# heliaxdev/ark-plonk

Measured on AMD Instinct MI355X. Metric: proofs/sec at 2^20 constraints (BLS12-381, KZG10); MSM G1-adds/s, higher is better.
Workload: dtype u32 limbs (256/384-bit Montgomery integers)

## Files before the change

### ark_plonk_amd/context.py

```python
from __future__ import annotations

import ctypes
import os
import threading

import numpy as np

from . import _lib
from ._lib import check, lib

_default = {}
_default_lock = threading.Lock()


def _is_torch(x) -> bool:
    return type(x).__module__.startswith("torch")


class Context:

    def __init__(self, device: int = 0, stream=None):
        self._h = ctypes.c_void_p()
        check(lib().zk_ctx_create(int(device), ctypes.byref(self._h)), "zk_ctx_create")
        self.device = int(device)
        self._stream_ptr = None
        self._stream_thread = None
        if stream is not None:
            self.set_stream(stream)
        lws = int(os.environ.get("LOCAL_WORLD_SIZE", "1") or 1)
        if lws > 1:
            cores = len(os.sched_getaffinity(0)) if hasattr(os, "sched_getaffinity") else (os.cpu_count() or 1)
            self.set_option("host_workers", max(0, min(15, cores // lws - 1)))

    def close(self):
        if getattr(self, "_h", None) is not None and self._h:
            lib().zk_ctx_destroy(self._h)
            self._h = None

    def __del__(self):
        try:
            self.close()
        except Exception:
            pass

    @property
    def handle(self):
        if not self._h:
            raise RuntimeError("context closed")
        return self._h

    def set_stream(self, stream):
        if stream is None:
            check(lib().zk_ctx_use_own_stream(self.handle), "zk_ctx_use_own_stream")
            self._stream_ptr = None
            self._stream_thread = None
            return
        ptr = int(getattr(stream, "cuda_stream", stream))
        if self._stream_ptr == ptr:
            return
        me = threading.get_ident()
        if self._stream_thread not in (None, me) and self._stream_ptr is not None:
            raise RuntimeError("Context is bound to another thread's stream: use one Context per thread and stream "
                               "(contexts are cheap and share CommitterKey handles via CommitterKey.with_ctx)")
        check(lib().zk_ctx_set_stream(self.handle, ctypes.c_void_p(ptr)), "zk_ctx_set_stream")
        self._stream_ptr = ptr
        self._stream_thread = me

    def use_torch_stream(self):
        import torch
        self.set_stream(torch.cuda.current_stream(self.device))

    def sync(self):
        check(lib().zk_ctx_sync(self.handle), "zk_ctx_sync")

    def set_msm_window(self, c: int):
        check(lib().zk_ctx_set_msm_window(self.handle, int(c)), "zk_ctx_set_msm_window")

    OPTIONS = ("msm_merge", "pre_vw", "pre_logg", "chunk_l", "long_rounds", "combine_sg", "pre_max_log_n", "mem_reserve_mb",
               "round_mem_limit_mb", "host_workers", "cache_verify")

    def set_option(self, key: str, value: int):
        check(lib().zk_ctx_set_option(self.handle, key.encode(), int(value)), f"zk_ctx_set_option({key})")

    def get_option(self, key: str) -> int:
        v = ctypes.c_int64()
        check(lib().zk_ctx_get_option(self.handle, key.encode(), ctypes.byref(v)), f"zk_ctx_get_option({key})")
        return v.value

    def round_mem_stats(self) -> dict:
        v = [ctypes.c_uint64() for _ in range(4)]
        check(lib().zk_round_mem_stats(self.handle, *[ctypes.byref(x) for x in v]), "zk_round_mem_stats")
        return {"early_closes": v[0].value, "set_bytes": v[1].value, "device_free": v[2].value, "device_total": v[3].value}

    def set_commit_cache(self, on: bool = True, capacity: int = 0):
        check(lib().zk_ctx_set_commit_cache(self.handle, 1 if on else 0, int(capacity)), "zk_ctx_set_commit_cache")

    def commit_cache_stats(self) -> dict:
        v = [ctypes.c_uint64() for _ in range(3)]
        check(lib().zk_commit_cache_stats(self.handle, *[ctypes.byref(x) for x in v]), "zk_commit_cache_stats")
        return {"hits": v[0].value, "misses": v[1].value, "entries": v[2].value}

    def set_residency_cache(self, on: bool = True, capacity_bytes: int = 0, max_vector_bytes: int = 0):
        check(lib().zk_ctx_set_residency_cache(self.handle, 1 if on else 0, int(capacity_bytes), int(max_vector_bytes)), "zk_ctx_set_residency_cache")

    def residency_cache_stats(self) -> dict:
        v = [ctypes.c_uint64() for _ in range(4)]
        check(lib().zk_residency_cache_stats(self.handle, *[ctypes.byref(x) for x in v]), "zk_residency_cache_stats")
        return {"hits": v[0].value, "misses": v[1].value, "entries": v[2].value, "bytes": v[3].value}

    def cache_verify_stats(self) -> dict:
        a, b = ctypes.c_uint64(), ctypes.c_uint64()
        check(lib().zk_cache_verify_stats(self.handle, ctypes.byref(a), ctypes.byref(b)), "zk_cache_verify_stats")
        return {"checked": a.value, "mismatches": b.value}

    def io_stats(self, reset: bool = False) -> dict:
        a, b = ctypes.c_uint64(), ctypes.c_uint64()
        check(lib().zk_io_stats(self.handle, ctypes.byref(a), ctypes.byref(b), 1 if reset else 0), "zk_io_stats")
        return {"h2d_bytes": a.value, "d2h_bytes": b.value}

    def set_staging(self, pinned_ring: bool = False):
        check(lib().zk_ctx_set_staging(self.handle, 1 if pinned_ring else 0), "zk_ctx_set_staging")

    def profile(self, on=True):
        check(lib().zk_profile_enable(self.handle, int(on)))

    def profile_reset(self):
        check(lib().zk_profile_reset(self.handle))

    def profile_get(self, name: str):
        t = ctypes.c_double()
        n = ctypes.c_uint64()
        check(lib().zk_profile_get(self.handle, name.encode(), ctypes.byref(t), ctypes.byref(n)))
        return t.value, n.value


def default_context(device: int = 0) -> Context:
    with _default_lock:
        ctx = _default.get(device)
        if ctx is None:
            ctx = Context(device)
            _default[device] = ctx
        return ctx


def ptr_of(x):
    if _is_torch(x):
        return ctypes.c_void_p(x.data_ptr())
    return ctypes.c_void_p(x.ctypes.data)


def as_host_u64(x, cols: int) -> np.ndarray:
    a = np.ascontiguousarray(x, dtype=np.uint64)
    if a.size % cols:
        raise ValueError(f"array size {a.size} not a multiple of {cols} limbs")
    return a.reshape(-1, cols)


def check_dev_tensor(t, cols: int, device: int):
    import torch
    if not t.is_cuda:
        raise ValueError("expected a CUDA/HIP tensor")
    if t.device.index != device:
# ... 9 lines not shown
```

### ark_plonk_amd/csrc/api_ctx.hip

```cpp
#include "api_internal.h"

#include <cstdio>

static thread_local char g_last_hip[256];

void zk_note_hip_error(hipError_t e, const char* what, const char* file, int line) {
    snprintf(g_last_hip, sizeof g_last_hip, "%s (%s) at %s:%d", hipGetErrorString(e), what, file, line);
    if (getenv("ZK_VERBOSE")) fprintf(stderr, "[ark_plonk_amd] HIP error: %s\n", g_last_hip);
}

ProfScope::ProfScope(zk_ctx* ctx, const char* nm) : ProfScope(ctx, nm, ctx->stream) {}
ProfScope::ProfScope(zk_ctx* ctx, const char* nm, hipStream_t stream) : c(ctx), name(nm), st(stream) {
    if (!c->profiling) return;
    if (c->profile_level == 2 && strcmp(nm, "msm_accumulate") != 0) return;
    auto take = [&]() -> hipEvent_t {
        if (!c->event_pool.empty()) {
            hipEvent_t e = c->event_pool.back();
            c->event_pool.pop_back();
            return e;
        }
        hipEvent_t e = nullptr;
        (void)hipEventCreate(&e);
        return e;
    };
// ... 65 lines not shown
    if (e != hipSuccess) {
        delete c;
        (void)hipSetDevice(prev);
        return ZK_ERR_HIP;
    }
    c->stream = c->own_stream;
    {
        const unsigned hc = std::thread::hardware_concurrency();
        c->tune.host_workers = hc > 16 ? 15 : hc > 1 ? (int)hc - 1 : 0;
        c->pool.reset(new HostPool((unsigned)c->tune.host_workers));
    }
    c->key_from_os = zk_process_key(c->ccache.digest_key);
    c->ccache.digest_key[0] ^= (uint64_t)(uintptr_t)c * 0x9E3779B97F4A7C15ull;
    for (int i = 0; i < ZK_MAX_JOBS && e == hipSuccess; ++i) e = hipEventCreateWithFlags(&c->ev_job[i], hipEventDisableTiming);
    (void)hipSetDevice(prev);
    if (e != hipSuccess) {
        zk_ctx_destroy(c);
        return ZK_ERR_HIP;
    }
    *out = c;
    return ZK_OK;
}

void zk_ctx_destroy(zk_ctx* c) {
    if (!c) return;
    {
        Guard g(c);
        (void)hipStreamSynchronize(c->stream);
        zk_prof_collect(c);
        for (hipEvent_t e : c->event_pool) (void)hipEventDestroy(e);
        ntt_ctx_free(c);
        DevBuf* bufs[] = {&c->io.a, &c->io.b, &c->msm_tmp, &c->stage_shared, &c->witness};
        for (DevBuf* b : bufs) b->release();
        for (int i = 0; i < ZK_MAX_JOBS; ++i) c->mb[i].release();
        res_clear(c);
        for (int i = 0; i < ZK_MAX_JOBS; ++i)
            if (c->ev_job[i]) (void)hipEventDestroy(c->ev_job[i]);
        if (c->round.ev) (void)hipEventDestroy(c->round.ev);
        if (c->pinned) (void)hipHostFree(c->pinned);
        if (c->pinned_small) (void)hipHostFree(c->pinned_small);
        if (c->round.pinned_jobs) (void)hipHostFree(c->round.pinned_jobs);
        zk_io_release(c);
        if (c->own_stream) (void)hipStreamDestroy(c->own_stream);
    }
    delete c;
}

static int switch_stream(zk_ctx* c, hipStream_t st) {
    Guard g(c);
    ZK_HIP_TRY(hipStreamSynchronize(c->stream));
    c->stream = st;
    return ZK_OK;
}
int zk_ctx_set_stream(zk_ctx* c, void* hip_stream) { return c ? switch_stream(c, (hipStream_t)hip_stream) : ZK_ERR_BAD_ARG; }
int zk_ctx_use_own_stream(zk_ctx* c) { return c ? switch_stream(c, c->own_stream) : ZK_ERR_BAD_ARG; }

int zk_ctx_sync(zk_ctx* c) {
    if (!c) return ZK_ERR_BAD_ARG;
    Guard g(c);
    ZK_HIP_TRY(hipStreamSynchronize(c->stream));
    return ZK_OK;
}

int zk_ctx_set_msm_window(zk_ctx* c, int w) {
    if (!c || w < 0 || w > 16 || w == 1) return ZK_ERR_BAD_ARG;
    Guard g(c);
    if (round_open(c)) return ZK_ERR_PENDING;
    c->msm_window = w;
    return ZK_OK;
}

static int* tune_field(zk_ctx* c, const char* key, int64_t* lo, int64_t* hi) {
    struct Row {
        const char* key;
        int ZkTune::*field;
        int64_t lo, hi;
    };
    static const Row rows[] = {
        {"msm_merge", &ZkTune::msm_merge, 0, 1},         {"pre_vw", &ZkTune::pre_vw, 0, 512},
        {"pre_logg", &ZkTune::pre_logg, -1, 5},          {"chunk_l", &ZkTune::chunk_l, 0, 1024},
        {"long_rounds", &ZkTune::long_rounds, 1, 16},    {"combine_sg", &ZkTune::combine_sg, 0, 4},
        {"pre_max_log_n", &ZkTune::pre_max_log_n, 0, 25}, {"mem_reserve_mb", &ZkTune::mem_reserve_mb, 0, 1 << 20},
        {"round_mem_limit_mb", &ZkTune::round_mem_limit_mb, 0, 1 << 20},
    };
    for (const Row& r : rows)
        if (strcmp(key, r.key) == 0) {
            *lo = r.lo;
            *hi = r.hi;
            return &(c->tune.*(r.field));
        }
    return nullptr;
}

int zk_ctx_set_option(zk_ctx* c, const char* key, int64_t value) {
    if (!c || !key) return ZK_ERR_BAD_ARG;
    Guard g(c);
    if (round_open(c)) return ZK_ERR_PENDING;
    int64_t lo = 0, hi = 0;
    if (strcmp(key, "cache_verify") == 0) {
        if (value < 0 || value > 1) return ZK_ERR_BAD_ARG;
        c->cache_verify = value != 0;
        return ZK_OK;
    }
    if (strcmp(key, "host_workers") == 0) {
        if (value < 0 || value > 63) return ZK_ERR_BAD_ARG;
        c->pool.reset(new HostPool((unsigned)value));
        c->tune.host_workers = (int)value;
        return ZK_OK;
    }
    int* f = tune_field(c, key, &lo, &hi);
    if (!f) return ZK_ERR_UNSUPPORTED;
    if (value < lo || value > hi) return ZK_ERR_BAD_ARG;
    if (f == &c->tune.pre_vw && value && (value < 8 || (value & (value - 1)))) return ZK_ERR_BAD_ARG;
    if (f == &c->tune.chunk_l && value && value < 8) return ZK_ERR_BAD_ARG;
    if (f == &c->tune.combine_sg && value == 3) return ZK_ERR_BAD_ARG;
    if (f == &c->tune.pre_max_log_n && value && value < 13) return ZK_ERR_BAD_ARG;
    *f = (int)value;
    return ZK_OK;
}

int zk_ctx_get_option(zk_ctx* c, const char* key, int64_t* value) {
    if (!c || !key || !value) return ZK_ERR_BAD_ARG;
    Guard g(c);
    int64_t lo = 0, hi = 0;
    if (strcmp(key, "host_workers") == 0) {
        *value = c->tune.host_workers;
        return ZK_OK;
    }
    if (strcmp(key, "cache_verify") == 0) {
        *value = c->cache_verify ? 1 : 0;
        return ZK_OK;
    }
    int* f = tune_field(c, key, &lo, &hi);
    if (!f) return ZK_ERR_UNSUPPORTED;
    *value = *f;
    return ZK_OK;
}

int zk_cache_verify_stats(zk_ctx* c, uint64_t* checked, uint64_t* mismatches) {
    if (!c) return ZK_ERR_BAD_ARG;
    Guard g(c);
    if (checked) *checked = c->verify_checked;
    if (mismatches) *mismatches = c->verify_mismatch;
    return ZK_OK;
}

int zk_profile_enable(zk_ctx* c, int on) {
    if (!c) return ZK_ERR_BAD_ARG;
    Guard g(c);
    c->profiling = on != 0;
    c->profile_level = on;
    return ZK_OK;
}
int zk_profile_reset(zk_ctx* c) {
    if (!c) return ZK_ERR_BAD_ARG;
    Guard g(c);
    ZK_HIP_TRY(hipStreamSynchronize(c->stream));
    zk_prof_collect(c);
    for (auto& kv : c->prof) {
        kv.second.total_ms = 0;
        kv.second.launches = 0;
    }
    return ZK_OK;
}
int zk_profile_get(zk_ctx* c, const char* name, double* total_ms, uint64_t* launches) {
    if (!c || !name) return ZK_ERR_BAD_ARG;
// ... 57 lines not shown
```

### ark_plonk_amd/csrc/ctx.h

```cpp
#pragma once
#include <hip/hip_runtime.h>
#include <cstring>
#include <cstdlib>
#include <atomic>
#include <list>
#include <map>
#include <mutex>
#include <shared_mutex>
#include <string>
#include <thread>
#include <condition_variable>
#include <functional>
#include <memory>
#include <vector>
#include <utility>

#include "../../include/ark_plonk_amd.h"
#include "curve_params.h"
#include "ec.cuh"
#include "fieldu.cuh"
#include "ecu.cuh"

typedef Fp<FrBls12_381Params> FrBls;
typedef Fp<FqBls12_381Params> FqBls;
// ... 131 lines not shown
    size_t need_for(size_t bytes) const { return bytes <= cap ? 0 : want_for(bytes); }
    int ensure(size_t bytes) {
        if (bytes <= cap) return ZK_OK;
        if (p) (void)hipFree(p);
        p = nullptr;
        cap = 0;
        size_t want = want_for(bytes);
        hipError_t e = hipMalloc(&p, want);
        if (e != hipSuccess) {
            p = nullptr;
            return ZK_ERR_OOM;
        }
        cap = want;
        return ZK_OK;
    }
    void release() {
        if (p) (void)hipFree(p);
        p = nullptr;
        cap = 0;
    }
};

struct MsmBufs {
    DevBuf counts, offsets, entries, buckets, part_pt, part_key, seg, seg2, seg3, win, tmp, scalars, stage, upload;
    int stage_of_job = 0;
    uint32_t acc_chunk_l = 0, acc_n_lanes = 0;
    void release() {
        release_work();
        scalars.release();
        upload.release();
    }
    void work_bufs(DevBuf* (&out)[12]) {
        DevBuf* all[12] = {&counts, &offsets, &entries, &buckets, &part_pt, &part_key, &seg, &seg2, &seg3, &win, &tmp, &stage};
        for (int i = 0; i < 12; ++i) out[i] = all[i];
    }
    size_t work_bytes() {
        DevBuf* w[12];
        work_bufs(w);
        size_t t = 0;
        for (DevBuf* b : w) t += b->cap;
        return t;
    }
    void release_work() {
        DevBuf* w[12];
        work_bufs(w);
        for (DevBuf* b : w) b->release();
    }
    void swap_work(MsmBufs& o) {
        DevBuf* a[12];
        DevBuf* b[12];
        work_bufs(a);
        o.work_bufs(b);
        for (int i = 0; i < 12; ++i) std::swap(*a[i], *b[i]);
    }
};

struct ProfEntry {
    double total_ms = 0;
    uint64_t launches = 0;
    std::vector<std::pair<hipEvent_t, hipEvent_t>> pending;
};

struct NttPlan {
    int curve = 0;
    uint32_t log_n = 0;
    bool inverse = false;
    int n_pass = 0;
    int s[4] = {0, 0, 0, 0};
    void* tw_inner[4] = {nullptr, nullptr, nullptr, nullptr};
    void* tw_pass[4] = {nullptr, nullptr, nullptr, nullptr};
    ~NttPlan() {
        for (int i = 0; i < 4; ++i)
            if (tw_pass[i]) (void)hipFree(tw_pass[i]);
    }
};

struct ZkTune {
    int msm_merge = 1;
    int pre_vw = 0;
    int pre_logg = -1;
    int chunk_l = 0;
    int long_rounds = 1;
    int combine_sg = 0;
    int pre_max_log_n = 0;
    int mem_reserve_mb = 1024;
    int round_mem_limit_mb = 0;
    int host_workers = -1;
};

struct zk_ctx {
    int device = 0;
    ZkTune tune;
    hipStream_t stream = nullptr;
    hipStream_t own_stream = nullptr;
    std::recursive_mutex mu;
    std::unique_ptr<HostPool> pool;
    int msm_window = 0;
    bool profiling = false;
    int profile_level = 0;
    std::map<std::string, ProfEntry> prof;
    std::vector<hipEvent_t> event_pool;

    std::map<uint64_t, NttPlan*> plans;
    std::map<uint64_t, void*> inner_tw;
    DevBuf ntt_work;
    DevBuf coset_pow[2];
    DevBuf coset_inv_pow[2];
    size_t coset_len[2] = {0, 0};
    size_t coset_inv_len[2] = {0, 0};

    MsmBufs mb[ZK_MAX_JOBS];
    hipEvent_t ev_job[ZK_MAX_JOBS] = {};
    void* pinned = nullptr;
    size_t pinned_cap = 0;
    void* pinned_small = nullptr;
    DevBuf msm_tmp;
    DevBuf stage_shared;
    DevBuf witness;

    struct HostIo {
        DevBuf a, b;
        hipStream_t copy_stream = nullptr;
        static constexpr int STAGE_SLOTS = 4;
        static constexpr size_t STAGE_BYTES = (size_t)8 << 20;
        void* stage_pin[STAGE_SLOTS] = {nullptr, nullptr, nullptr, nullptr};
        hipEvent_t stage_ev[STAGE_SLOTS] = {nullptr, nullptr, nullptr, nullptr};
        bool stage_busy[STAGE_SLOTS] = {false, false, false, false};
        int stage_next = 0;
        hipEvent_t ev_up[ZK_MAX_JOBS] = {};
        uint64_t h2d_bytes = 0, d2h_bytes = 0;
        int staging_mode = 0;
    } io;

    struct CommitCache {
        struct Entry {
            uint64_t srs_id;
            uint64_t n;
            uint32_t kind;
            uint64_t dig[4];
            uint64_t xy[ZK_MAX_AFFINE64];
            uint8_t inf;
        };
        bool on = false;
        size_t cap = 64;
        std::list<Entry> entries;
        uint64_t hits = 0, misses = 0;
        DevBuf digest_dev;
        uint64_t digest_key[4] = {0, 0, 0, 0};
    } ccache;

    struct Residency {
        struct Entry {
            size_t bytes = 0;
            uint64_t dig[4] = {0, 0, 0, 0};
            bool valid = false;
            uint64_t epoch = 0;
            uint64_t born = 0;
            DevBuf buf;
        };
        bool on = false;
        size_t cap = (size_t)2 << 30, max_vec = (size_t)64 << 20, bytes = 0;
        std::list<Entry> entries;
        std::vector<DevBuf> free_bufs;
        uint64_t epoch = 0, hits = 0, misses = 0;
        std::vector<unsigned char> verify_host;
    } res;
// ... 141 lines not shown
```

### ark_plonk_amd/csrc/ecq.cuh

```cuda
#pragma once
#include "ecu.cuh"

template <class F>
ZK_D F quad_xor(const F& v, int mask) {
    F r;
#pragma unroll
    for (int i = 0; i < F::NL; ++i) r.v[i] = __shfl_xor(v.v[i], mask, 64);
    return r;
}
template <class F>
ZK_D F quad_bcast(const F& v, uint32_t src_role) {
    const int src = (int)((__lane_id() & ~3u) | src_role);
    F r;
#pragma unroll
    for (int i = 0; i < F::NL; ++i) r.v[i] = __shfl(v.v[i], src, 64);
    return r;
}
template <class F>
ZK_D F fsel(bool c, const F& a, const F& b) {
    F r;
#pragma unroll
    for (int i = 0; i < F::NL; ++i) r.v[i] = c ? a.v[i] : b.v[i];
    return r;
}
ZK_D bool quad_flag(bool f, uint32_t src_role) {
    const unsigned long long b = __ballot(f);
    return (b >> ((__lane_id() & ~3u) | src_role)) & 1ull;
}

template <class F>
ZK_D XYZZu<F> quad_gather(const F& c) {
    XYZZu<F> p;
    p.x = quad_bcast(c, 0);
    p.y = quad_bcast(c, 1);
    p.zz = quad_bcast(c, 2);
    p.zzz = quad_bcast(c, 3);
    return p;
}
template <class F>
ZK_D F quad_pick(const XYZZu<F>& p, uint32_t role) {
    return role == 0 ? p.x : role == 1 ? p.y : role == 2 ? p.zz : p.zzz;
}
template <class F>
ZK_D bool quad_is_inf(const F& c, uint32_t role) {
    return quad_flag(role == 2 && c.limbs_zero(), 2);
}

template <class F>
ZK_D F qdbl(const F& p, uint32_t role);

template <class F>
ZK_D F qadd(const F& p, const F& q, uint32_t role) {
    const bool p_inf = quad_is_inf(p, role), q_inf = quad_is_inf(q, role);
    const F m1 = F::mul(p, quad_xor(q, 2));
    const F d = F::sub8(quad_xor(m1, 2), m1);
    const bool lo = role < 2;
    const F m2 = F::mul(fsel(lo, d, p), fsel(lo, d, q));
    const F bc_u1 = quad_bcast(m1, 0), bc_pp = quad_bcast(m2, 0);
    const F m3 = F::mul(role == 0 ? d : role == 1 ? bc_u1 : m2, fsel(role == 0, m2, bc_pp));
    const F bc_ppp = quad_bcast(m3, 0);
    const F x3 = F::sub_sum3(m2, bc_ppp, m3, m3);
    const bool r1 = role == 1;
    const F m4 = F::dot2(fsel(r1, d, m2), fsel(r1, F::sub16(m3, x3), bc_ppp), fsel(r1, F::neg16(m1), F::zero()), bc_ppp);
    const F x3_from_role1 = quad_xor(x3, 1);
    F res = role == 0 ? x3_from_role1 : role == 2 ? m3 : m4;
    const bool same_x = quad_flag(role == 2 && m3.is_zero_mod_reduced(), 2);
    const bool same_y = quad_flag(role == 1 && m2.is_zero_mod_reduced(), 1);
    const bool slow = same_x && !p_inf && !q_inf;
    if (__any(slow)) {
        const F twice = qdbl<F>(p, role);
        if (slow) res = same_y ? twice : F::zero();
    }
    if (q_inf) res = p;
    if (p_inf) res = q;
    return res;
}

template <class F>
ZK_D F qdbl(const F& p, uint32_t role) {
    const bool p_inf = quad_is_inf(p, role);
    const F a1 = fsel(role == 1, F::dbl(p), p);
    const F m1 = F::mul(a1, a1);
    const F bc_v = quad_bcast(m1, 1);
    const F m2 = F::mul(a1, bc_v);
    const F mm = F::add3(m1, m1, m1);
    const F bc_w = quad_bcast(m2, 1);
    const bool r0 = role == 0;
    const F m3 = F::mul(fsel(r0, mm, p), fsel(r0, mm, bc_w));
    const F x3 = F::sub8(m3, F::dbl(m2));
    const F m4 = F::dot2(mm, F::sub16(m2, x3), bc_w, F::neg16(quad_bcast(p, 1)));
    const F y3_from_role0 = quad_xor(m4, 1);
    F res = role == 0 ? x3 : role == 1 ? y3_from_role0 : role == 2 ? m2 : m3;
    if (p_inf) res = p;
    return res;
}
```

### ark_plonk_amd/csrc/msm_reduce.hip

```cpp
#include "msm_common.cuh"
#include "ecq.cuh"

namespace {


ZK_D uint64_t partial_slot(uint32_t t, uint32_t ta, uint32_t s, uint32_t L) {
    return (t == ta && (s % L) != 0) ? 2ull * t + 1 : 2ull * t;
}

template <class F>
ZK_D XYZZu<F> wave_sum(XYZZu<F> acc) {
#pragma unroll 1
    for (int d = 32; d >= 1; d >>= 1) {
        XYZZu<F> o;
#pragma unroll
        for (int i = 0; i < F::NL; ++i) {
            o.x.v[i] = __shfl_down(acc.x.v[i], d, 64);
            o.y.v[i] = __shfl_down(acc.y.v[i], d, 64);
            o.zz.v[i] = __shfl_down(acc.zz.v[i], d, 64);
            o.zzz.v[i] = __shfl_down(acc.zzz.v[i], d, 64);
        }
        acc = XYZZu<F>::add(acc, o);
    }
    return acc;
// ... 242 lines not shown
    auto bucket = [&](int i) -> F {
        const uint32_t bi = w * g.B + sg * G + (uint32_t)i;
        F v = F::zero();
        if (live && (!offsets || offsets[bi + 1] != offsets[bi])) v = ld_coord<F>(buckets, bi, role);
        return v;
    };
    F nv = bucket((int)G - 1);
#pragma unroll 1
    for (int i = (int)G - 1; i >= 0; --i) {
        const F v = nv;
        if (i > 0) nv = bucket(i - 1);
        run = qadd<F>(run, v, role);
        acc = qadd<F>(acc, run, role);
    }
    if (live) {
        st_coord<F>(seg_run, id, role, run);
        st_coord<F>(seg_acc, id, role, acc);
    }
}

template <class F, int MAXT>
__global__ void __launch_bounds__(MAXT) __attribute__((amdgpu_waves_per_eu(MAXT / 256, MAXT / 256))) msm_win_finish_q(RJobs jobs, MsmGeom g, uint32_t raw) {
    extern __shared__ uint4 sh[];
    const void* seg_run = jobs.seg_run[blockIdx.y];
    const void* seg_acc = jobs.seg_acc[blockIdx.y];
    uint32_t* win_out = jobs.win_s[blockIdx.y];
    uint32_t* tot_out = jobs.win_t[blockIdx.y];
    const uint32_t w = blockIdx.x, u = threadIdx.x >> 2, role = threadIdx.x & 3;
    const uint32_t T = blockDim.x >> 2;
    F R = F::zero(), Y = F::zero();
    if (u < g.ns) {
        R = ld_coord<F>(seg_run, (uint64_t)w * g.ns + u, role);
        Y = ld_coord<F>(seg_acc, (uint64_t)w * g.ns + u, role);
    }
    st_coord<F>(sh, u, role, R);
    for (uint32_t d = 1; d < T; d <<= 1) {
        __syncthreads();
        F o = F::zero();
        if (u + d < T) o = ld_coord<F>(sh, u + d, role);
        __syncthreads();
        R = qadd<F>(R, o, role);
        st_coord<F>(sh, u, role, R);
    }
    const bool r_inf = quad_is_inf(R, role);
    if (tot_out && u == 0) {
        if (raw) {
            st_coord<F>(tot_out, w, role, r_inf ? F::zero() : R);
        } else {
            uint32_t* o = tot_out + (size_t)w * 4 * F::SAT + role * F::SAT;
            if (r_inf) {
                for (int i = 0; i < F::SAT; ++i) o[i] = 0;
            } else {
                R.to_sat(o);
            }
        }
    }
    F Qm = R;
    for (uint32_t k = 0; k < g.logG; ++k) Qm = qdbl<F>(Qm, role);
    F Z = qadd<F>(Y, u >= 1 ? Qm : F::zero(), role);
    __syncthreads();
    st_coord<F>(sh, u, role, Z);
    for (uint32_t d = T / 2; d >= 1; d >>= 1) {
        __syncthreads();
        if (u < d) {
            Z = qadd<F>(Z, ld_coord<F>(sh, u + d, role), role);
            st_coord<F>(sh, u, role, Z);
        }
    }
    const bool z_inf = quad_is_inf(Z, role);
    if (u == 0) {
        if (raw) {
            st_coord<F>(win_out, w, role, z_inf ? F::zero() : Z);
        } else {
            uint32_t* o = win_out + (size_t)w * 4 * F::SAT + role * F::SAT;
            if (z_inf) {
                for (int i = 0; i < F::SAT; ++i) o[i] = 0;
            } else {
                Z.to_sat(o);
            }
        }
    }
}

template <class F>
__global__ void __launch_bounds__(256) __attribute__((amdgpu_waves_per_eu(1, 2))) msm_node_reduce_q(RJobs jobs, uint32_t n_out, uint32_t logk, uint32_t logm) {
    const void* in_run = jobs.seg_run[blockIdx.y];
    const void* in_acc = jobs.seg_acc[blockIdx.y];
    void* out_run = jobs.win_s[blockIdx.y];
    void* out_acc = jobs.win_t[blockIdx.y];
    const uint32_t tid = blockIdx.x * blockDim.x + threadIdx.x;
    const uint32_t id = tid >> 2, role = tid & 3;
    const bool live = id < n_out;
    const uint32_t K = 1u << logk;
    const uint64_t first = (uint64_t)(live ? id : 0) * K;
    F run = F::zero(), wsum = F::zero(), asum = F::zero();
#pragma unroll 1
    for (int j = (int)K - 1; j >= 1; --j) {
        run = qadd<F>(run, live ? ld_coord<F>(in_run, first + (uint32_t)j, role) : F::zero(), role);
        wsum = qadd<F>(wsum, run, role);
        asum = qadd<F>(asum, live ? ld_coord<F>(in_acc, first + (uint32_t)j, role) : F::zero(), role);
    }
    run = qadd<F>(run, live ? ld_coord<F>(in_run, first, role) : F::zero(), role);
    asum = qadd<F>(asum, live ? ld_coord<F>(in_acc, first, role) : F::zero(), role);
    for (uint32_t t = 0; t < logm; ++t) wsum = qdbl<F>(wsum, role);
    asum = qadd<F>(asum, wsum, role);
    if (live) {
        st_coord<F>(out_run, id, role, run);
        st_coord<F>(out_acc, id, role, asum);
    }
}

template <class F>
__global__ void __launch_bounds__(256) __attribute__((amdgpu_waves_per_eu(1, 2))) g1_sum_winsums_q(const void* all, uint32_t ranks, uint32_t n_pts ,
                                                                                                     uint32_t logq, uint32_t* out_sat) {
    extern __shared__ uint4 sh[];
    const uint32_t Q = 1u << logq;
    const uint32_t quad = threadIdx.x >> 2, role = threadIdx.x & 3;
    const uint32_t per_block = (blockDim.x >> 2) >> logq;
    const uint32_t k = blockIdx.x * per_block + (quad >> logq), j = quad & (Q - 1);
    const bool live = k < n_pts;
    F acc = F::zero();
#pragma unroll 1
    for (uint32_t r = j; r < ranks; r += Q) acc = qadd<F>(acc, live ? ld_coord<F>(all, (uint64_t)r * n_pts + k, role) : F::zero(), role);
    for (uint32_t d = Q >> 1; d >= 1; d >>= 1) {
        st_coord<F>(sh, quad, role, acc);
        __syncthreads();
        const F o = j < d ? ld_coord<F>(sh, quad + d, role) : F::zero();
        __syncthreads();
        acc = qadd<F>(acc, o, role);
    }
    const bool inf = quad_is_inf(acc, role);
    if (live && j == 0) {
        uint32_t* o = out_sat + (size_t)k * 4 * F::SAT + role * F::SAT;
        if (inf) {
            for (int i = 0; i < F::SAT; ++i) o[i] = 0;
        } else {
            acc.to_sat(o);
        }
    }
}

template <class F>
int launch_win_finish_q(dim3 grid, uint32_t chains, hipStream_t st, const RJobs& jobs, const MsmGeom& g, uint32_t raw) {
    constexpr size_t PT = (size_t)4 * Store<F>::WORDS * 4;
    const size_t shmem = (size_t)chains * PT;
    if (chains <= 128) {
        if (shmem > 48 * 1024)
            ZK_HIP_TRY(hipFuncSetAttribute((const void*)msm_win_finish_q<F, 512>, hipFuncAttributeMaxDynamicSharedMemorySize, (int)shmem));
        hipLaunchKernelGGL((msm_win_finish_q<F, 512>), grid, dim3(4 * chains), shmem, st, jobs, g, raw);
    } else if (chains <= 256) {
        if (shmem > 48 * 1024)
            ZK_HIP_TRY(hipFuncSetAttribute((const void*)msm_win_finish_q<F, 1024>, hipFuncAttributeMaxDynamicSharedMemorySize, (int)shmem));
        hipLaunchKernelGGL((msm_win_finish_q<F, 1024>), grid, dim3(4 * chains), shmem, st, jobs, g, raw);
    } else {
        return ZK_ERR_UNSUPPORTED;
    }
    return ZK_OK;
}

template <class F>
int queue_reduce(zk_ctx* c, const RJobs& jobs, uint32_t n_jobs, uint32_t nb, const MsmGeom& gr, hipStream_t st, bool queues_cleared = false,
                 uint32_t raw = 0 ) {
    constexpr size_t PT = (size_t)4 * Store<F>::WORDS * 4;
    ProfScope ps(c, "msm_reduce", st);
    const int T = 128;
    int rc;
    if (!queues_cleared)
        for (uint32_t k = 0; k < n_jobs; ++k) ZK_HIP_TRY(hipMemsetAsync(jobs.q[k], 0, 8, st));
    const bool quad = gr.logq == 0 && gr.ns <= 256;
    if (n_jobs <= 2) {
        if (quad) {
            unsigned blocks = (unsigned)(((uint64_t)nb * 4 + 255) / 256);
            hipLaunchKernelGGL(msm_combine_q<F>, dim3(blocks, n_jobs), dim3(256), 0, st, jobs, nb);
        } else {
            unsigned blocks = (unsigned)(((uint64_t)nb * 4 + T - 1) / T);
            hipLaunchKernelGGL((msm_combine<F, 4>), dim3(blocks, n_jobs), dim3(T), 0, st, jobs, nb);
        }
    } else {
        const int sg = c->tune.combine_sg ? c->tune.combine_sg : 1;
        if (sg == 4) {
            unsigned blocks = (unsigned)(((uint64_t)nb * 4 + T - 1) / T);
            hipLaunchKernelGGL((msm_combine<F, 4>), dim3(blocks, n_jobs), dim3(T), 0, st, jobs, nb);
        } else if (sg == 2) {
            unsigned blocks = (unsigned)(((uint64_t)nb * 2 + T - 1) / T);
            hipLaunchKernelGGL((msm_combine<F, 2>), dim3(blocks, n_jobs), dim3(T), 0, st, jobs, nb);
        } else {
            unsigned blocks = (unsigned)(((uint64_t)nb + T - 1) / T);
            hipLaunchKernelGGL((msm_combine<F, 1>), dim3(blocks, n_jobs), dim3(T), 0, st, jobs, nb);
        }
    }
    hipLaunchKernelGGL(msm_combine_wave<F>, dim3(256, n_jobs), dim3(256), 0, st, jobs);
    hipLaunchKernelGGL(msm_combine_block<F>, dim3(64, n_jobs), dim3(256), 4 * PT, st, jobs, nb);
    if (quad) {
        unsigned sblocks = (unsigned)(((uint64_t)gr.W * gr.ns * 4 + 255) / 256);
        hipLaunchKernelGGL(msm_seg_reduce_q<F>, dim3(sblocks, n_jobs), dim3(256), 0, st, jobs, gr);
        uint32_t chains = 1;
        while (chains < gr.ns) chains <<= 1;
        size_t shmem = (size_t)chains * PT;
        if ((rc = launch_win_finish_q<F>(dim3(gr.W, n_jobs), chains, st, jobs, gr, raw))) return rc;
    } else {
        if (raw) return ZK_ERR_UNSUPPORTED;
        unsigned sblocks = (gr.W * gr.ns + T - 1) / T;
        hipLaunchKernelGGL(msm_seg_reduce<F>, dim3(sblocks, n_jobs), dim3(T), 0, st, jobs, gr);
        size_t shmem = 256 * PT;
        if (shmem > 48 * 1024)
            ZK_HIP_TRY(hipFuncSetAttribute((const void*)msm_win_finish<F>, hipFuncAttributeMaxDynamicSharedMemorySize, (int)shmem));
        hipLaunchKernelGGL(msm_win_finish<F>, dim3(gr.W, n_jobs), dim3(256), shmem, st, jobs, gr);
    }
    ZK_HIP_TRY(hipGetLastError());
    return ZK_OK;
}

template <class F>
int queue_reduce_wide(zk_ctx* c, const RJobs& jobs, uint32_t n_jobs, uint32_t nb, void* const* d_vw, void* const* d_seg3, void* const* d_seg2,
                      char* h_out, size_t h_stride, hipStream_t st) {
    constexpr size_t PT = (size_t)4 * Store<F>::WORDS * 4;
    ProfScope ps(c, "msm_reduce", st);
    int rc;
    const uint32_t VW = nb / WIDE_VB;
    if (VW == 0 || VW > 2048) return ZK_ERR_UNSUPPORTED;
    {
        const int T = 128;
        if (n_jobs <= 2) {
            unsigned blocks = (unsigned)(((uint64_t)nb * 4 + 255) / 256);
            hipLaunchKernelGGL(msm_combine_q<F>, dim3(blocks, n_jobs), dim3(256), 0, st, jobs, nb);
        } else {
            unsigned blocks = (unsigned)(((uint64_t)nb + T - 1) / T);
            hipLaunchKernelGGL((msm_combine<F, 1>), dim3(blocks, n_jobs), dim3(T), 0, st, jobs, nb);
        }
        hipLaunchKernelGGL(msm_combine_wave<F>, dim3(256, n_jobs), dim3(256), 0, st, jobs);
        hipLaunchKernelGGL(msm_combine_block<F>, dim3(64, n_jobs), dim3(256), 4 * PT, st, jobs, nb);
    }
    const uint32_t n1 = nb >> WIDE_LOGG1, n2 = n1 >> WIDE_LOGK2;
    {
        MsmGeom g1;
        memset(&g1, 0, sizeof g1);
        g1.W = 1;
        g1.B = nb;
        g1.nb = nb;
        g1.logG = WIDE_LOGG1;
        g1.ns = n1;
        const int T = 128;
        unsigned sblocks = (unsigned)(((uint64_t)n1 + T - 1) / T);
        hipLaunchKernelGGL(msm_seg_reduce<F>, dim3(sblocks, n_jobs), dim3(T), 0, st, jobs, g1);
    }
    RJobs j2 = jobs;
    for (uint32_t k = 0; k < n_jobs; ++k) {
        j2.win_s[k] = (uint32_t*)d_seg2[k];
        j2.win_t[k] = (uint32_t*)((char*)d_seg2[k] + (size_t)n2 * PT);
    }
    {
        unsigned blocks = (unsigned)(((uint64_t)n2 * 4 + 255) / 256);
        hipLaunchKernelGGL(msm_node_reduce_q<F>, dim3(blocks, n_jobs), dim3(256), 0, st, j2, n2, WIDE_LOGK2, WIDE_LOGG1);
    }
    RJobs j3 = jobs;
    MsmGeom gv;
    memset(&gv, 0, sizeof gv);
    gv.W = VW;
    gv.B = WIDE_VB;
    gv.nb = nb;
    gv.logG = WIDE_LOGG1 + WIDE_LOGK2;
    gv.ns = WIDE_CHAINS;
    for (uint32_t k = 0; k < n_jobs; ++k) {
        j3.seg_run[k] = d_seg2[k];
        j3.seg_acc[k] = (char*)d_seg2[k] + (size_t)n2 * PT;
        j3.win_s[k] = (uint32_t*)d_vw[k];
        j3.win_t[k] = (uint32_t*)((char*)d_vw[k] + (size_t)VW * PT);
    }
    {
        if ((rc = launch_win_finish_q<F>(dim3(VW, n_jobs), WIDE_CHAINS, st, j3, gv, 1u))) return rc;
    }
    MsmGeom g4;
    memset(&g4, 0, sizeof g4);
    g4.W = 1;
    g4.B = VW;
    g4.nb = VW;
    g4.logG = VW <= 4 ? 0 : VW <= 1024 ? 2 : 3;
    g4.ns = VW >> g4.logG;
    if (g4.ns == 0 || g4.ns > 256) return ZK_ERR_UNSUPPORTED;
    RJobs j4;
    memset(&j4, 0, sizeof j4);
    const size_t PHB = h_stride / 4;
    for (uint32_t k = 0; k < n_jobs; ++k)
        for (uint32_t a = 0; a < 2; ++a) {
            const uint32_t j = 2 * k + a;
            j4.buckets[j] = (char*)d_vw[k] + (size_t)a * VW * PT;
            j4.offsets[j] = nullptr;
            j4.seg_run[j] = (char*)d_seg3[k] + (size_t)a * 2 * g4.ns * PT;
            j4.seg_acc[j] = (char*)d_seg3[k] + ((size_t)a * 2 + 1) * g4.ns * PT;
            j4.win_s[j] = (uint32_t*)(h_out + (size_t)k * h_stride + (size_t)a * 2 * PHB);
            j4.win_t[j] = (uint32_t*)(h_out + (size_t)k * h_stride + ((size_t)a * 2 + 1) * PHB);
        }
    {
        unsigned sblocks = (unsigned)(((uint64_t)g4.ns * 4 + 255) / 256);
        hipLaunchKernelGGL(msm_seg_reduce_q<F>, dim3(sblocks, 2 * n_jobs), dim3(256), 0, st, j4, g4);
        uint32_t chains = 1;
        while (chains < g4.ns) chains <<= 1;
        if ((rc = launch_win_finish_q<F>(dim3(1, 2 * n_jobs), chains, st, j4, g4, 0u))) return rc;
    }
    ZK_HIP_TRY(hipGetLastError());
    return ZK_OK;
}

template <class Cv>
int pre_queue_reduce(zk_ctx* c, const PrePlan* pls, MsmBufs* const* mbs, uint32_t n_jobs, void* h_win, hipStream_t st, void* const* d_winsums) {
    typedef typename Cv::FqU F;
    constexpr size_t PT = (size_t)4 * Store<F>::WORDS * 4;
    RJobs jobs;
    memset(&jobs, 0, sizeof jobs);
    const PrePlan& p0 = pls[0];
    if (d_winsums && !pre_partial_dev_ok(p0)) return ZK_ERR_UNSUPPORTED;
    for (uint32_t k = 0; k < n_jobs; ++k) {
        MsmBufs& mb = *mbs[k];
        jobs.part_pt[k] = mb.part_pt.p;
        jobs.offsets[k] = (const uint32_t*)mb.offsets.p;
        jobs.buckets[k] = mb.buckets.p;
        jobs.q[k] = (uint32_t*)mb.part_key.p + PRE_Q_OFF;
        jobs.seg_run[k] = mb.seg.p;
        jobs.seg_acc[k] = (char*)mb.seg.p + (p0.wide_red ? (size_t)(p0.g.B >> WIDE_LOGG1) : (size_t)p0.gv.W * p0.gv.ns) * PT;
        if (d_winsums) {
            jobs.win_s[k] = (uint32_t*)d_winsums[k];
            jobs.win_t[k] = (uint32_t*)((char*)d_winsums[k] + (size_t)p0.gv.W * PT);
        } else {
            jobs.win_s[k] = (uint32_t*)((char*)h_win + (size_t)k * p0.win_bytes);
            jobs.win_t[k] = jobs.win_s[k] + (size_t)p0.gv.W * 4 * F::SAT;
        }
        jobs.L[k] = mb.acc_chunk_l;
        jobs.lanes[k] = mb.acc_n_lanes;
        jobs.nbk[k] = p0.g1.nb;
    }
    if (p0.wide_red) {
        void* d_vw[MAX_JOBS];
        void* d_seg3[MAX_JOBS];
        void* d_seg2[MAX_JOBS];
        for (uint32_t k = 0; k < n_jobs; ++k) {
            d_vw[k] = mbs[k]->win.p;
            d_seg3[k] = mbs[k]->seg3.p;
            d_seg2[k] = mbs[k]->seg2.p;
        }
        return queue_reduce_wide<F>(c, jobs, n_jobs, p0.g1.nb, d_vw, d_seg3, d_seg2, (char*)h_win, p0.win_bytes, st);
    }
    return queue_reduce<F>(c, jobs, n_jobs, p0.g1.nb, p0.gv, st, true, d_winsums ? 1u : 0u);
}

}

int ZK_SYM(queue_reduce)(zk_ctx* c, const RJobs& jobs, uint32_t n_jobs, uint32_t nb, const MsmGeom& gr, hipStream_t st, bool queues_cleared, uint32_t raw) {
    return queue_reduce<CurveSel::FqU>(c, jobs, n_jobs, nb, gr, st, queues_cleared, raw);
}
int ZK_SYM(pre_queue_reduce)(zk_ctx* c, const PrePlan* pls, MsmBufs* const* mbs, uint32_t n_jobs, void* h_win, hipStream_t st, void* const* d_winsums) {
    return pre_queue_reduce<CurveSel>(c, pls, mbs, n_jobs, h_win, st, d_winsums);
}
int ZK_SYM(queue_sum_winsums)(zk_ctx* c, const void* d_all, uint32_t ranks, uint32_t n_pts, void* h_out, hipStream_t st) {
    typedef CurveSel::FqU F;
    ProfScope ps(c, "msm_sum_winsums", st);
    constexpr size_t PT = (size_t)4 * Store<F>::WORDS * 4;
    uint32_t logq = 0;
    while (logq < 4 && (2u << logq) < ranks) ++logq;
    const uint32_t per_block = 64u >> logq;
    hipLaunchKernelGGL(g1_sum_winsums_q<F>, dim3((n_pts + per_block - 1) / per_block), dim3(256), 64 * PT, st, d_all, ranks, n_pts, logq, (uint32_t*)h_out);
    ZK_HIP_TRY(hipGetLastError());
    return ZK_OK;
}
```

Baseline: 12.18.

## Add scan-based big-bucket combine and fused bucket/segment reduce for precomputed MSM

For the precomputed-table MSM path, a new msm_combine_big kernel replaces the queue-based wave/block combine kernels. Each wave scans a range of buckets, handles large buckets inline, and defers the very largest to a per-block list reduced by the whole block. Optional fused_form kernels fold the partial-sum combine for small buckets directly into the segment running-sum reduce, skipping the separate combine and seg_reduce launches. The quad-lane EC add/double code also swaps ternaries for fsel selects to avoid divergence. The trade-off is per-block serialisation on big buckets and overflow handling when the big list fills.

Result: no change. 12.17 (-0.1%).

```diff
diff --git a/ark_plonk_amd/context.py b/ark_plonk_amd/context.py
--- a/ark_plonk_amd/context.py
+++ b/ark_plonk_amd/context.py
@@ -77,7 +77,7 @@
         check(lib().zk_ctx_set_msm_window(self.handle, int(c)), "zk_ctx_set_msm_window")
 
     OPTIONS = ("msm_merge", "pre_vw", "pre_logg", "chunk_l", "long_rounds", "combine_sg", "pre_max_log_n", "mem_reserve_mb",
-               "round_mem_limit_mb", "host_workers", "cache_verify")
+               "round_mem_limit_mb", "host_workers", "cache_verify", "msm_split_reduce", "fused_form")
 
     def set_option(self, key: str, value: int):
         check(lib().zk_ctx_set_option(self.handle, key.encode(), int(value)), f"zk_ctx_set_option({key})")
diff --git a/ark_plonk_amd/csrc/api_ctx.hip b/ark_plonk_amd/csrc/api_ctx.hip
--- a/ark_plonk_amd/csrc/api_ctx.hip
+++ b/ark_plonk_amd/csrc/api_ctx.hip
@@ -171,6 +171,7 @@
         {"long_rounds", &ZkTune::long_rounds, 1, 16},    {"combine_sg", &ZkTune::combine_sg, 0, 4},
         {"pre_max_log_n", &ZkTune::pre_max_log_n, 0, 25}, {"mem_reserve_mb", &ZkTune::mem_reserve_mb, 0, 1 << 20},
         {"round_mem_limit_mb", &ZkTune::round_mem_limit_mb, 0, 1 << 20},
+        {"msm_split_reduce", &ZkTune::msm_split_reduce, 0, 1}, {"fused_form", &ZkTune::fused_form, 0, 2},
     };
     for (const Row& r : rows)
         if (strcmp(key, r.key) == 0) {
diff --git a/ark_plonk_amd/csrc/ctx.h b/ark_plonk_amd/csrc/ctx.h
--- a/ark_plonk_amd/csrc/ctx.h
+++ b/ark_plonk_amd/csrc/ctx.h
@@ -237,6 +237,8 @@
     int chunk_l = 0;
     int long_rounds = 1;
     int combine_sg = 0;
+    int msm_split_reduce = 0;
+    int fused_form = 0;
     int pre_max_log_n = 0;
     int mem_reserve_mb = 1024;
     int round_mem_limit_mb = 0;
diff --git a/ark_plonk_amd/csrc/ecq.cuh b/ark_plonk_amd/csrc/ecq.cuh
--- a/ark_plonk_amd/csrc/ecq.cuh
+++ b/ark_plonk_amd/csrc/ecq.cuh
@@ -57,22 +57,22 @@
     const bool lo = role < 2;
     const F m2 = F::mul(fsel(lo, d, p), fsel(lo, d, q));
     const F bc_u1 = quad_bcast(m1, 0), bc_pp = quad_bcast(m2, 0);
-    const F m3 = F::mul(role == 0 ? d : role == 1 ? bc_u1 : m2, fsel(role == 0, m2, bc_pp));
+    const F m3 = F::mul(fsel(role == 0, d, fsel(role == 1, bc_u1, m2)), fsel(role == 0, m2, bc_pp));
     const F bc_ppp = quad_bcast(m3, 0);
     const F x3 = F::sub_sum3(m2, bc_ppp, m3, m3);
     const bool r1 = role == 1;
     const F m4 = F::dot2(fsel(r1, d, m2), fsel(r1, F::sub16(m3, x3), bc_ppp), fsel(r1, F::neg16(m1), F::zero()), bc_ppp);
     const F x3_from_role1 = quad_xor(x3, 1);
-    F res = role == 0 ? x3_from_role1 : role == 2 ? m3 : m4;
+    F res = fsel(role == 0, x3_from_role1, fsel(role == 2, m3, m4));
     const bool same_x = quad_flag(role == 2 && m3.is_zero_mod_reduced(), 2);
     const bool same_y = quad_flag(role == 1 && m2.is_zero_mod_reduced(), 1);
     const bool slow = same_x && !p_inf && !q_inf;
     if (__any(slow)) {
         const F twice = qdbl<F>(p, role);
-        if (slow) res = same_y ? twice : F::zero();
+        res = fsel(slow, fsel(same_y, twice, F::zero()), res);
     }
-    if (q_inf) res = p;
-    if (p_inf) res = q;
+    res = fsel(q_inf, p, res);
+    res = fsel(p_inf, q, res);
     return res;
 }
 
@@ -90,7 +90,6 @@
     const F x3 = F::sub8(m3, F::dbl(m2));
     const F m4 = F::dot2(mm, F::sub16(m2, x3), bc_w, F::neg16(quad_bcast(p, 1)));
     const F y3_from_role0 = quad_xor(m4, 1);
-    F res = role == 0 ? x3 : role == 1 ? y3_from_role0 : role == 2 ? m2 : m3;
-    if (p_inf) res = p;
-    return res;
+    F res = fsel(role == 0, x3, fsel(role == 1, y3_from_role0, fsel(role == 2, m2, m3)));
+    return fsel(p_inf, p, res);
 }
diff --git a/ark_plonk_amd/csrc/msm_reduce.hip b/ark_plonk_amd/csrc/msm_reduce.hip
--- a/ark_plonk_amd/csrc/msm_reduce.hip
+++ b/ark_plonk_amd/csrc/msm_reduce.hip
@@ -348,6 +348,179 @@
     }
 }
 
+constexpr uint32_t BIG_BLOCKS = 256;
+constexpr uint32_t BIG_LIST = 62;
+template <class F>
+__global__ void __launch_bounds__(256) msm_combine_big(RJobs jobs, uint32_t nb) {
+    __shared__ uint4 sh[4 * 4 * Store<F>::U4];
+    __shared__ uint32_t big[BIG_LIST + 2];
+    const void* part_pt = jobs.part_pt[blockIdx.y];
+    const uint32_t* offsets = jobs.offsets[blockIdx.y];
+    void* buckets = jobs.buckets[blockIdx.y];
+    const uint32_t L = chunk_len(offsets[jobs.nbk[blockIdx.y]], jobs.lanes[blockIdx.y], jobs.L[blockIdx.y]);
+    const uint32_t u = threadIdx.x, lane = u & 63;
+    if (u == 0) big[0] = 0;
+    __syncthreads();
+    const uint32_t per_wave = (nb + gridDim.x * 4 - 1) / (gridDim.x * 4);
+    const uint32_t b0 = (blockIdx.x * 4 + (u >> 6)) * per_wave;
+    const uint32_t b1 = b0 + per_wave < nb ? b0 + per_wave : nb;
+    for (uint32_t base = b0; base < b1; base += 64) {
+        const uint32_t b = base + lane;
+        uint32_t p = 0, s = 0;
+        if (b < b1) {
+            s = offsets[b];
+            const uint32_t e = offsets[b + 1];
+            if (e != s) p = (e - 1) / L - s / L + 1;
+        }
+        unsigned long long m = __ballot(p > COMBINE_SMALL);
+        while (m) {
+            const int src = __ffsll((long long)m) - 1;
+            m &= m - 1;
+            const uint32_t bb = base + (uint32_t)src;
+            const uint32_t ps = __shfl(p, src, 64), ss = __shfl(s, src, 64);
+            if (ps > COMBINE_MEDIUM) {
+                uint32_t slot = 0;
+                if (lane == 0) slot = atomicAdd(&big[0], 1u);
+                slot = __shfl(slot, 0, 64);
+                if (slot < BIG_LIST) {
+                    if (lane == 0) big[1 + slot] = bb;
+                    continue;
+                }
+            }
+            const uint32_t ta = ss / L, tb = ta + ps - 1;
+            XYZZu<F> acc = XYZZu<F>::infinity();
+            for (uint32_t t = ta + lane; t <= tb; t += 64) acc = XYZZu<F>::add(acc, ld_xyzz<F>(part_pt, partial_slot(t, ta, ss, L)));
+            acc = wave_sum<F>(acc);
+            if (lane == 0) st_xyzz<F>(buckets, bb, acc);
+        }
+    }
+    __syncthreads();
+    const uint32_t nl = big[0] < BIG_LIST ? big[0] : BIG_LIST;
+    for (uint32_t h = 0; h < nl; ++h) {
+        const uint32_t b = big[1 + h];
+        const uint32_t s = offsets[b], e = offsets[b + 1];
+        const uint32_t ta = s / L, tb = (e - 1) / L;
+        XYZZu<F> acc = XYZZu<F>::infinity();
+        for (uint32_t t = ta + u; t <= tb; t += 256) acc = XYZZu<F>::add(acc, ld_xyzz<F>(part_pt, partial_slot(t, ta, s, L)));
+        acc = wave_sum<F>(acc);
+        __syncthreads();
+        if (lane == 0) st_xyzz<F>(sh, u >> 6, acc);
+        __syncthreads();
+        if (u == 0) {
+            for (uint32_t w = 1; w < 4; ++w) acc = XYZZu<F>::add(acc, ld_xyzz<F>(sh, w));
+            st_xyzz<F>(buckets, b, acc);
+        }
+    }
+}
+
+struct BucketTerms {
+    uint32_t np, ta;
+    uint64_t head;
+    bool from_partials;
+};
+ZK_D BucketTerms bucket_terms(const uint32_t* offsets, uint32_t bi, uint32_t L) {
+    BucketTerms d;
+    d.np = 0;
+    d.ta = 0;
+    d.head = bi;
+    d.from_partials = false;
+    const uint32_t s = offsets[bi], e = offsets[bi + 1];
+    if (e != s) {
+        d.ta = s / L;
+        const uint32_t p = (e - 1) / L - d.ta + 1;
+        d.np = 1;
+        if (p > 1 && p <= COMBINE_SMALL) {
+            d.np = p;
+            d.head = partial_slot(d.ta, d.ta, s, L);
+            d.from_partials = true;
+        }
+    }
+    return d;
+}
+
+template <class F>
+__global__ void __launch_bounds__(256) __attribute__((amdgpu_waves_per_eu(1, 2))) msm_fused_reduce_q(RJobs jobs, MsmGeom g) {
+    const void* part_pt = jobs.part_pt[blockIdx.y];
+    const void* buckets = jobs.buckets[blockIdx.y];
+    const uint32_t* offsets = jobs.offsets[blockIdx.y];
+    void* seg_run = jobs.seg_run[blockIdx.y];
+    void* seg_acc = jobs.seg_acc[blockIdx.y];
+    const uint32_t L = chunk_len(offsets[jobs.nbk[blockIdx.y]], jobs.lanes[blockIdx.y], jobs.L[blockIdx.y]);
+    const uint32_t tid = blockIdx.x * blockDim.x + threadIdx.x;
+    const uint32_t id = tid >> 2, role = tid & 3;
+    const bool live = id < g.W * g.ns;
+    const uint32_t w = live ? id / g.ns : 0, sg = live ? id % g.ns : 0;
+    const uint32_t G = 1u << g.logG;
+    const uint32_t first = w * g.B + sg * G;
+    F run = F::zero(), acc = F::zero();
+    BucketTerms nd;
+    auto head_of = [&](int i) -> F {
+        nd = bucket_terms(offsets, first + (uint32_t)i, L);
+        if (!live) nd.np = 0;
+        return nd.np ? ld_coord<F>(nd.from_partials ? part_pt : buckets, nd.head, role) : F::zero();
+    };
+    F nv = head_of((int)G - 1);
+#pragma unroll 1
+    for (int i = (int)G - 1; i >= 0; --i) {
+        F b = nv;
+        const BucketTerms d = nd;
+        if (i > 0) nv = head_of(i - 1);
+        const uint32_t more = d.from_partials ? d.np - 1 : 0;
+        uint32_t steps = more;
+#pragma unroll
+        for (int x = 32; x >= 4; x >>= 1) {
+            const uint32_t o = __shfl_xor(steps, x, 64);
+            steps = o > steps ? o : steps;
+        }
+        F pv = more ? ld_coord<F>(part_pt, 2ull * (d.ta + 1), role) : F::zero();
+#pragma unroll 1
+        for (uint32_t k = 1; k <= steps; ++k) {
+            const F v = pv;
+            pv = k < more ? ld_coord<F>(part_pt, 2ull * (d.ta + k + 1), role) : F::zero();
+            b = qadd<F>(b, v, role);
+        }
+        run = qadd<F>(run, b, role);
+        acc = qadd<F>(acc, run, role);
+    }
+    if (live) {
+        st_coord<F>(seg_run, id, role, run);
+        st_coord<F>(seg_acc, id, role, acc);
+    }
+}
+
+template <class F>
+__global__ void __launch_bounds__(128) msm_fused_reduce(RJobs jobs, MsmGeom g) {
+    const void* part_pt = jobs.part_pt[blockIdx.y];
+    const void* buckets = jobs.buckets[blockIdx.y];
+    const uint32_t* offsets = jobs.offsets[blockIdx.y];
+    void* seg_run = jobs.seg_run[blockIdx.y];
+    void* seg_acc = jobs.seg_acc[blockIdx.y];
+    const uint32_t L = chunk_len(offsets[jobs.nbk[blockIdx.y]], jobs.lanes[blockIdx.y], jobs.L[blockIdx.y]);
+    const uint32_t id = blockIdx.x * blockDim.x + threadIdx.x;
+    if (id >= g.W * g.ns) return;
+    const uint32_t w = id / g.ns, sg = id % g.ns;
+    const uint32_t G = 1u << g.logG;
+    const uint32_t first = w * g.B + sg * G;
+    XYZZu<F> run = XYZZu<F>::infinity(), acc = XYZZu<F>::infinity();
+    BucketTerms nd = bucket_terms(offsets, first + G - 1, L);
+#pragma unroll 1
+    for (int i = (int)G - 1; i >= 0; --i) {
+        const BucketTerms d = nd;
+        if (i > 0) nd = bucket_terms(offsets, first + (uint32_t)i - 1, L);
+        if (d.np) {
+            XYZZu<F> b = ld_xyzz<F>(d.from_partials ? part_pt : buckets, d.head);
+            if (d.from_partials) {
+#pragma unroll 1
+                for (uint32_t k = 1; k < d.np; ++k) b = XYZZu<F>::add(b, ld_xyzz<F>(part_pt, 2ull * (d.ta + k)));
+            }
+            run = XYZZu<F>::add(run, b);
+        }
+        acc = XYZZu<F>::add(acc, run);
+    }
+    st_xyzz<F>(seg_run, id, run);
+    st_xyzz<F>(seg_acc, id, acc);
+}
+
 template <class F>
 __global__ void __launch_bounds__(256) __attribute__((amdgpu_waves_per_eu(1, 2))) msm_node_reduce_q(RJobs jobs, uint32_t n_out, uint32_t logk, uint32_t logm) {
     const void* in_run = jobs.seg_run[blockIdx.y];
@@ -426,11 +599,30 @@
 
 template <class F>
 int queue_reduce(zk_ctx* c, const RJobs& jobs, uint32_t n_jobs, uint32_t nb, const MsmGeom& gr, hipStream_t st, bool queues_cleared = false,
-                 uint32_t raw = 0 ) {
+                 uint32_t raw = 0 ,
+                 bool table = false) {
     constexpr size_t PT = (size_t)4 * Store<F>::WORDS * 4;
     ProfScope ps(c, "msm_reduce", st);
     const int T = 128;
     int rc;
+    const bool scan = table && !c->tune.msm_split_reduce && gr.logq == 0 && gr.ns <= 256 && nb == gr.W * gr.B;
+    if (scan) {
+        hipLaunchKernelGGL(msm_combine_big<F>, dim3(BIG_BLOCKS, n_jobs), dim3(256), 0, st, jobs, nb);
+        if (c->tune.fused_form) {
+            if (c->tune.fused_form == 2) {
+                unsigned sblocks = (gr.W * gr.ns + T - 1) / T;
+                hipLaunchKernelGGL(msm_fused_reduce<F>, dim3(sblocks, n_jobs), dim3(T), 0, st, jobs, gr);
+            } else {
+                unsigned sblocks = (unsigned)(((uint64_t)gr.W * gr.ns * 4 + 255) / 256);
+                hipLaunchKernelGGL(msm_fused_reduce_q<F>, dim3(sblocks, n_jobs), dim3(256), 0, st, jobs, gr);
+            }
+            uint32_t chains = 1;
+            while (chains < gr.ns) chains <<= 1;
+            if ((rc = launch_win_finish_q<F>(dim3(gr.W, n_jobs), chains, st, jobs, gr, raw))) return rc;
+            ZK_HIP_TRY(hipGetLastError());
+            return ZK_OK;
+        }
+    }
     if (!queues_cleared)
         for (uint32_t k = 0; k < n_jobs; ++k) ZK_HIP_TRY(hipMemsetAsync(jobs.q[k], 0, 8, st));
     const bool quad = gr.logq == 0 && gr.ns <= 256;
@@ -455,8 +647,10 @@
             hipLaunchKernelGGL((msm_combine<F, 1>), dim3(blocks, n_jobs), dim3(T), 0, st, jobs, nb);
         }
     }
-    hipLaunchKernelGGL(msm_combine_wave<F>, dim3(256, n_jobs), dim3(256), 0, st, jobs);
-    hipLaunchKernelGGL(msm_combine_block<F>, dim3(64, n_jobs), dim3(256), 4 * PT, st, jobs, nb);
+    if (!scan) {
+        hipLaunchKernelGGL(msm_combine_wave<F>, dim3(256, n_jobs), dim3(256), 0, st, jobs);
+        hipLaunchKernelGGL(msm_combine_block<F>, dim3(64, n_jobs), dim3(256), 4 * PT, st, jobs, nb);
+    }
     if (quad) {
         unsigned sblocks = (unsigned)(((uint64_t)gr.W * gr.ns * 4 + 255) / 256);
         hipLaunchKernelGGL(msm_seg_reduce_q<F>, dim3(sblocks, n_jobs), dim3(256), 0, st, jobs, gr);
@@ -606,7 +800,7 @@
         }
         return queue_reduce_wide<F>(c, jobs, n_jobs, p0.g1.nb, d_vw, d_seg3, d_seg2, (char*)h_win, p0.win_bytes, st);
     }
-    return queue_reduce<F>(c, jobs, n_jobs, p0.g1.nb, p0.gv, st, true, d_winsums ? 1u : 0u);
+    return queue_reduce<F>(c, jobs, n_jobs, p0.g1.nb, p0.gv, st, true, d_winsums ? 1u : 0u, true);
 }
 
 }
```
